# Phaken/graph-embeddings

Hardware: AMD Instinct MI355X
Metric: GloVe pair-updates/sec at dim=200 (higher is better)
Workload: dtype f32

## Files before the change

graph-embeddings_amd/csrc/ge_layout.h:

```cpp
#pragma once
#include "ge_common.h"
#include <vector>

namespace ge {

constexpr int LAYOUT_CHUNK = 128;

struct LayoutRequest {
    int32_t V, row_begin, row_end;
    int64_t N;
    int32_t cost;
    double  xmax;
    int32_t hot_columns;
    double  hot_theta;
    double  stale_budget;
    int32_t flush_every;
    int32_t workers;
    int32_t shared_rows;
    int32_t pack_rows;
    bool    want_hub_index;
    bool    device_input;
    int32_t tile_g;
    int32_t tile_force;
    int32_t tile_workers;
    int32_t panels;
    int32_t panel_blocks;
    int32_t blocks;
};

struct BlockedLayout {
    int32_t *bA = nullptr, *bB = nullptr, *border = nullptr;
    double  *L = nullptr;
    float   *W = nullptr;
    int32_t *cstart = nullptr;
    int32_t *cmeta = nullptr;
    int32_t *tcols = nullptr;
    int32_t *tlim = nullptr;
    int64_t P = 0, n_chunks = 0, n_hchunks = 0;
    int64_t n_tchunks = 0, tile_nnz = 0, tile_visits = 0;
    int32_t tile_g = 0, tile_cols = 0, n_tgroups = 0;
    int32_t *prow0 = nullptr, *prows = nullptr, *ppos = nullptr;
    int64_t n_pchunks = 0, panel_nnz = 0, panel_visits = 0;
// ... 20 lines not shown
```

graph-embeddings_amd/csrc/glove.hip:

```cpp

#include "ge_common.h"
#include "ge_coo.h"
#include "ge_glove_internal.h"
#include "ge_javarand.h"
#include "ge_cost.h"
#include "ge_exact.h"
#include "ge_strata.h"
#include "ge_wave.h"
#include "ge_layout.h"

#include <algorithm>
#include <cmath>
#include <cstdlib>
#include <cstring>
#include <chrono>
#include <memory>
#include <new>
#include <type_traits>
#include <vector>

namespace {

enum { ORDER_IDENTITY = 0, ORDER_PERM = 1, ORDER_BIJECTION = 2 };

// ... 191 lines not shown
    __builtin_amdgcn_s_waitcnt(0xC07F);
    __builtin_amdgcn_s_barrier();
    asm volatile("" ::: "memory");
}

constexpr int RUN_CHUNK = 128;
constexpr int KEY_PAD = 0x7FFFFFFF;
constexpr int TILE_N_AFTER = 4;

enum { PAIR_MEM = 0, PAIR_LDS = 1 };
struct PanelLink {
    const int32_t *rows;
    int32_t n_rows;
    int32_t lag;
    float *nextA, *nextB;
};
template <int G, int SRC, int SINK>
__device__ __forceinline__ void tile_chunk(const GloveParams &p, const int32_t c_lo, const int32_t c_len, const int32_t grp,
                                           float *const setA, float *const setB, float *const tr_c, float *const tr_g,
                                           int32_t *const stg, double &cost_acc, const PanelLink &pl, const int lane) {
    constexpr bool PIPE = SRC == PAIR_LDS || SINK == PAIR_LDS;
    constexpr int N_AFTER = SINK == PAIR_MEM ? TILE_N_AFTER : TILE_N_AFTER - 2;
    static_assert(G >= 2 && G <= 8, "two to eight resident columns");
    const int32_t D = p.D, DS = p.DS;
    const uint32_t row_bytes = (uint32_t)p.RW * 4u;
    const int bl_lane = (D / 4) & 63;
    const bool inr = lane * 4 < D, is_bl = lane == bl_lane;
    const float lr = p.lr;
    constexpr int IMG_G = 256;
    auto rl = [&](float v) { return __builtin_bit_cast(float, __builtin_amdgcn_readlane(__builtin_bit_cast(int, v), bl_lane)); };

    int s_lane = lane;
    asm volatile("" : "+v"(s_lane));
#pragma unroll
    for (int q = 0; q < 2; ++q) {
        const int e = q * 64 + s_lane;
        if (e < c_len) {
// ... 6 lines not shown
    __builtin_amdgcn_fence(__ATOMIC_RELEASE, "wavefront");
    __builtin_amdgcn_wave_barrier();
    __builtin_amdgcn_fence(__ATOMIC_ACQUIRE, "wavefront");
    auto staged = [&](int what, int e) { return rfl(stg[what * RUN_CHUNK + rfl(e)]); };
    auto row_at = [&](int e) { return staged(0, e); };

    auto request = [&](float *img, int32_t row, bool live) {
        const uint32_t rbytes = live ? row_bytes : 0u;
        load_to_lds<16>(make_rsrc(p.focus + (int64_t)row * DS, rbytes), img, lane * 16);
        load_to_lds<16>(make_rsrc(p.gsf + (int64_t)row * DS, rbytes), img + IMG_G, lane * 16);
        asm volatile("" ::: "memory");
    };
    int32_t n_row = 0;
    if constexpr (!PIPE) n_row = row_at(0);
    else if constexpr (SRC == PAIR_MEM) n_row = rfl(pl.rows[0]);
    if constexpr (SRC == PAIR_MEM) request(setA, n_row, true);

    float4 a[G], ga[G], a0[G], ga0[G];
    int32_t col[G], lim[G], cnt[G];
    auto ctx_rsrc = [&](int32_t c) { return make_rsrc(p.context + (int64_t)(c < 0 ? 0 : c) * DS, c < 0 ? 0u : row_bytes); };
    auto gsc_rsrc = [&](int32_t c) { return make_rsrc(p.gsc + (int64_t)(c < 0 ? 0 : c) * DS, c < 0 ? 0u : row_bytes); };
#pragma unroll
    for (int s = 0; s < G; ++s) {
        col[s] = rfl(p.tcols[(int64_t)grp * G + s]); lim[s] = rfl(p.tlim[(int64_t)grp * G + s]); cnt[s] = 0;
    }
#pragma unroll
    for (int s = 0; s < G; ++s) {
        a[s] = buf_load<4, AUX_SC1>(ctx_rsrc(col[s]), lane * 16);
        ga[s] = buf_load<4, AUX_SC1>(gsc_rsrc(col[s]), lane * 16);
    }
#pragma unroll
// ... 90 lines not shown
        bool more;
        if constexpr (!PIPE) {
            row = n_row;
            nxt = pos + 1;
            for (;;) {
                more = nxt < c_len;
                n_row = more ? row_at(nxt) : 0;
                if (!more || n_row != row) break;
                ++nxt;
            }
        } else {
            row = rfl(pl.rows[ri]);
            nxt = pos;
            while (nxt < c_len && row_at(nxt) == row) ++nxt;
            more = ri + 1 < pl.n_rows;
            if constexpr (SRC == PAIR_MEM) n_row = more ? rfl(pl.rows[ri + 1]) : 0;
        }
        const float *const img = decltype(CUR)::value ? setB : setA;
        if constexpr (SRC == PAIR_MEM) {
            request(decltype(CUR)::value ? setA : setB, n_row, more);
            __builtin_amdgcn_s_waitcnt(wait_vmcnt(N_AFTER));
        }
        asm volatile("" ::: "memory");
        b = *reinterpret_cast<const float4 *>(img + lane * 4);
        gb = *reinterpret_cast<const float4 *>(img + IMG_G + lane * 4);
        bb = rl(b.x); gbb = rl(gb.x);
        for (int e = pos; e < nxt; ++e) {
            const int s = staged(1, e);
            const float w = __builtin_bit_cast(float, staged(2, e));
            const unsigned lo = (unsigned)rfl(stg[3 * RUN_CHUNK + 2 * rfl(e)]), hi = (unsigned)rfl(stg[3 * RUN_CHUNK + 2 * rfl(e) + 1]);
            const double l = __builtin_bit_cast(double, ((unsigned long long)hi << 32) | lo);
            update(s, w, l);
        }
        float4 ob = b, ogb = gb;
        if (!inr) {
            ob = float4{0.0f, 0.0f, 0.0f, 0.0f}; ogb = ob;
            if (is_bl) { ob.x = bb; ogb.x = gbb; }
        }
        if constexpr (SINK == PAIR_MEM) {
            buf_store<4>(ob, make_rsrc(p.focus + (int64_t)row * DS, row_bytes), lane * 16);
// ... 18 lines not shown
        for (int ri = 0; ri < pl.n_rows; ri += 2) {
            walk_row(IMG_A, ri);
            lds_barrier();
            if (ri + 1 < pl.n_rows) {
                walk_row(IMG_B, ri + 1);
                lds_barrier();
            }
        }
        for (int i = pl.lag; i < 3; ++i) lds_barrier();
    }
#pragma nounroll
    for (int s = 0; s < G; ++s)
        for_slot(s, [&](auto S) { constexpr int q = decltype(S)::value; if (cnt[q] > 0) publish(col[q], a[q], ga[q], a0[q], ga0[q]); });
}

template <int VW, int NCH, int OPT, bool EMB16, bool FAT, int TG, bool PANELS = false>
__device__ __forceinline__ void epoch_walk(const GloveParams &p, const int32_t n_workers) {
    using VT = typename Vec<VW>::T;
    static_assert(!EMB16 || VW == 4, "bf16 embeddings need dim % 4 == 0");
    constexpr bool MOM = OPT != GE_OPT_ADAGRAD;
    int tid = (int)threadIdx.x;
    uint32_t sr_state = 0x9E3779B9u * (uint32_t)(threadIdx.x + 1) + (uint32_t)blockIdx.x * 0x85EBCA6Bu + p.bij_key[0];
    auto emb_rsrc = [&](float *base, int64_t id) {
        if constexpr (EMB16) return make_rsrc(reinterpret_cast<uint16_t *>(base) + id * p.ES, (uint32_t)p.D * 2u);
        else return make_rsrc(base + id * p.DS, (uint32_t)p.RW * 4u);
    };
    auto emb_load = [&](__amdgpu_buffer_rsrc_t rs, int q) -> VT {
        if constexpr (EMB16) return widen_bf16x4(buf_load<2, AUX_SC1>(rs, ((tid & 63) + q * 64) * 8));
        else return buf_load<VW, AUX_SC1>(rs, ((tid & 63) + q * 64) * VW * 4);
    };
    auto emb_store = [&](VT v, __amdgpu_buffer_rsrc_t rs, int q) {
// ... 59 lines not shown
            }
            __syncthreads();
            const int32_t tk = rfl(s_pticket);
            if (tk < 0) break;
            uint32_t x = (uint32_t)tk;
            do { x = bij_mix(x, p.pbij_mask, p.pbij_shift, p.bij_key); } while (x >= (uint32_t)n_pchunks);
            const int32_t pc = rfl((int)x);
            const int32_t r0 = rfl(p.prow0[pc]), nr = rfl(p.prow0[pc + 1]) - r0;
            if (tid < nr) s_prow[tid] = p.prows[r0 + tid];
            if (tid + 256 < nr && tid + 256 < 4 * RUN_CHUNK) s_prow[tid + 256] = p.prows[r0 + tid + 256];
            if (tid == 0) s_pn = nr < 4 * RUN_CHUNK ? nr : 4 * RUN_CHUNK;
            __syncthreads();
            const int32_t *const pp = p.ppos + (int64_t)pc * 9;
            const int32_t grp = rfl(pp[0]) * 4 + wib, c_lo = rfl(pp[1 + 2 * wib]), c_len = rfl(pp[2 + 2 * wib]);
            const int nx = wib < 3 ? wib + 1 : 0;
            const PanelLink pl{s_prow, rfl(s_pn), wib, s_setA + nx * SET_FLOATS, s_setB + nx * SET_FLOATS};
            float *const tr_c = s_tr[wib][0], *const tr_g = s_tr[wib][1];
            float *const setA = s_setA + wib * SET_FLOATS, *const setB = s_setB + wib * SET_FLOATS;
            if (wib == 0) tile_chunk<TG, PAIR_MEM, PAIR_LDS>(p, c_lo, c_len, grp, setA, setB, tr_c, tr_g, s_stage[wib], cost_acc, pl, tid & 63);
            else if (wib < 3) tile_chunk<TG, PAIR_LDS, PAIR_LDS>(p, c_lo, c_len, grp, setA, setB, tr_c, tr_g, s_stage[wib], cost_acc, pl, tid & 63);
            else tile_chunk<TG, PAIR_LDS, PAIR_MEM>(p, c_lo, c_len, grp, setA, setB, tr_c, tr_g, s_stage[wib], cost_acc, pl, tid & 63);
        }
        s_pcost[wib] = cost_acc;
        __syncthreads();
        if (wib == 0) cost_acc = ((s_pcost[0] + s_pcost[1]) + s_pcost[2]) + s_pcost[3];
        else cost_acc = 0.0;
        continue;
    }
    if (wave >= n_workers) continue;
    }
    const int lane = tid & 63;
    float *const setA = s_setA + (tid >> 6) * SET_FLOATS, *const setB = s_setB + (tid >> 6) * SET_FLOATS;
    bool inr[NCH];
#pragma unroll
// ... 379 lines not shown
    }
    if ((tid & 63) == 0 && cost_acc != 0.0) atomicAdd(p.cost_out, cost_acc);
}

template <int VW, int NCH, int OPT, bool EMB16, bool FAT>
__global__ __launch_bounds__(256, (NCH == 1 && VW == 4 && OPT == GE_OPT_ADAGRAD) ? 5 : 1) void k_adagrad_runs(GloveParams p, int32_t n_workers) {
    epoch_walk<VW, NCH, OPT, EMB16, FAT, 0>(p, n_workers);
}
constexpr int TILE_G = 4;
template <int G>
__global__ __launch_bounds__(256, 3) void k_epoch_tiles(GloveParams p, int32_t n_workers) {
    epoch_walk<4, 1, GE_OPT_ADAGRAD, false, true, G>(p, n_workers);
}
__global__ __launch_bounds__(256, 3) void k_epoch_panels(GloveParams p, int32_t n_workers) {
    epoch_walk<4, 1, GE_OPT_ADAGRAD, false, true, TILE_G, true>(p, n_workers);
}

__global__ __launch_bounds__(256) void k_probe_records(float *tab, int64_t rows, int64_t ds, int32_t rec_bytes, int32_t iters, uint32_t seed) {
    const int lane = threadIdx.x & 63;
    uint32_t x = (uint32_t)(blockIdx.x * 4 + (threadIdx.x >> 6)) * 0x9E3779B1u + seed;
    for (int it = 0; it < iters; ++it) {
        x = x * 1664525u + 1013904223u;
        const int64_t r = (int64_t)(((uint64_t)(x >> 4) * (uint64_t)rows) >> 28);
        const __amdgpu_buffer_rsrc_t rs = make_rsrc(tab + r * ds, (uint32_t)rec_bytes);
        float4 v[4];
#pragma unroll
        for (int q = 0; q < 4; ++q) v[q] = buf_load<4, AUX_SC1>(rs, (lane + q * 64) * 16);
#pragma unroll
        for (int q = 0; q < 4; ++q) buf_store<4>(v[q], rs, (lane + q * 64) * 16);
    }
// ... 298 lines not shown
    if (cfg->cost != GE_COST_GLOVE && cfg->cost != GE_COST_PGLOVE) return ge::fail(GE_ERR_ARG, "Invalid cost function %d", cfg->cost);
    if (cfg->opt < GE_OPT_ADAGRAD || cfg->opt > GE_OPT_AMSGRAD) return ge::fail(GE_ERR_ARG, "Invalid optimization method %d", cfg->opt);
    if (cfg->threads < 1) return ge::fail(GE_ERR_ARG, "threads must be >= 1");
    if (cfg->mode != GE_MODE_HOGWILD && cfg->mode != GE_MODE_DETERMINISTIC && cfg->mode != GE_MODE_STRATIFIED) return ge::fail(GE_ERR_ARG, "invalid mode %d", cfg->mode);
    if (cfg->strata < 0 || cfg->strata > 2048) return ge::fail(GE_ERR_ARG, "strata must lie in [0, 2048] (got %d; 0 = the default for the matrix)", cfg->strata);
    if (cfg->strata != 0 && cfg->mode != GE_MODE_STRATIFIED) return ge::fail(GE_ERR_ARG, "strata = %d needs mode = GE_MODE_STRATIFIED", cfg->strata);
    if (cfg->shuffle < GE_SHUFFLE_JAVA || cfg->shuffle > GE_SHUFFLE_NONE) return ge::fail(GE_ERR_ARG, "invalid shuffle %d", cfg->shuffle);
    if (cfg->mode == GE_MODE_STRATIFIED && cfg->shuffle == GE_SHUFFLE_JAVA)
        return ge::fail(GE_ERR_ARG, "the stratified mode cannot follow a global Fisher-Yates order: shuffle must be device or none");
    if (cfg->workers < -(1 << 20)) return ge::fail(GE_ERR_ARG, "workers out of range");
    if (cfg->emb_dtype != GE_DTYPE_F32 && cfg->emb_dtype != GE_DTYPE_BF16) return ge::fail(GE_ERR_ARG, "invalid emb_dtype %d", cfg->emb_dtype);
    const bool emb16 = cfg->emb_dtype == GE_DTYPE_BF16;
    if (emb16 && (cfg->mode != GE_MODE_HOGWILD || cfg->shuffle != GE_SHUFFLE_DEVICE || cfg->opt != GE_OPT_ADAGRAD || cfg->dim % 4 != 0))
        return ge::fail(GE_ERR_ARG, "bf16 embeddings need mode=hogwild, shuffle=device, opt=adagrad and dim %% 4 == 0 (the reference path is fp32)");
    if (cfg->hot_columns < GE_HOT_AUTO || cfg->hot_columns > GE_HOT_ALL) return ge::fail(GE_ERR_ARG, "invalid hot_columns %d", cfg->hot_columns);
    if (cfg->hot_theta < 0 || cfg->stale_budget < 0 || cfg->flush_every < 0 || cfg->blocks_per_cu < 0 || (cfg->layout_flags & ~511) != 0)
        return ge::fail(GE_ERR_ARG, "invalid tuning fields (hot_theta %g, stale_budget %g, flush_every %d, blocks_per_cu %d, layout_flags %d)",
                        (double)cfg->hot_theta, (double)cfg->stale_budget, cfg->flush_every, cfg->blocks_per_cu, cfg->layout_flags);
    int32_t rb = cfg->row_begin, re = cfg->row_end;
    if (rb == 0 && re == 0) re = cfg->vocab_size;
    if (rb < 0 || re > cfg->vocab_size || rb >= re) return ge::fail(GE_ERR_ARG, "invalid row range [%d,%d)", rb, re);
    const bool will_block = cfg->mode == GE_MODE_HOGWILD && cfg->shuffle == GE_SHUFFLE_DEVICE;
    if (!will_block)
        for (int64_t k = 0; k < cfg->nnz; ++k) {
            if (I[k] < rb || I[k] >= re) return ge::fail(GE_ERR_ARG, "I[%lld]=%d outside owned rows [%d,%d)", (long long)k, I[k], rb, re);
            if (J[k] < 0 || J[k] >= cfg->vocab_size) return ge::fail(GE_ERR_ARG, "J[%lld]=%d outside [0,%d)", (long long)k, J[k], cfg->vocab_size);
        }
    *rb_out = rb; *re_out = re;
    return GE_OK;
}

// ... 104 lines not shown
    blocks = std::min<int64_t>(blocks, std::max<int64_t>(1, N / 2048 / groups_per_block));
    w.blocks = (int)std::max<int64_t>(blocks, 1);
    w.workers = w.blocks * 4;
    if (cfg.workers > 0) {
        w.workers = (int)std::min<int64_t>(cfg.workers, (int64_t)h->num_cus * 32);
        w.blocks = (w.workers + 3) / 4;
    } else if (cfg.workers < 0) {
        w.blocks = (int)std::max<int64_t>(1, (int64_t)w.blocks - (-(int64_t)cfg.workers + 3) / 4);
        w.workers = w.blocks * 4;
    }
    return w;
}
void take_plan(ge_glove *h, const WorkerPlan &w) { h->hw_blocks_per_cu = w.blocks_per_cu; h->hw_blocks = w.blocks; h->hw_workers = w.workers; }
void plan_workers(ge_glove *h) { take_plan(h, plan_workers_of(h, h->hw.fn)); }

bool tiles_forced(const ge_glove_cfg &cfg) {
    const bool panels_asked = (cfg.layout_flags & (GE_LAYOUT_HUB_PANELS | GE_LAYOUT_NO_HUB_PANELS)) == GE_LAYOUT_HUB_PANELS;
    return (cfg.layout_flags & GE_LAYOUT_HUB_TILES) != 0 || (panels_asked && cfg.nnz < ((int64_t)1 << 25));
}
bool tiles_possible(const ge_glove *h) {
    const ge_glove_cfg &cfg = h->cfg;
    if (cfg.layout_flags & GE_LAYOUT_NO_HUB_TILES) return false;
    if (h->emb16 || cfg.opt != GE_OPT_ADAGRAD || !h->hw.fat || h->hw.vw != 4 || h->hw.nch != 1) return false;
    if (cfg.shuffle != GE_SHUFFLE_DEVICE || h->rows != cfg.vocab_size) return false;
    return tiles_forced(cfg) || cfg.nnz >= ((int64_t)1 << 25);
}
bool panels_possible(const ge_glove *h) {
    const ge_glove_cfg &cfg = h->cfg;
    if ((cfg.layout_flags & GE_LAYOUT_NO_HUB_PANELS) || !tiles_possible(h)) return false;
    return (cfg.layout_flags & GE_LAYOUT_HUB_PANELS) != 0 || cfg.nnz >= ((int64_t)1 << 25);
}

ge_status plan_epoch_layout(ge_glove *h, const int32_t *I, const int32_t *J, const float *X, bool device_input) {
    const ge_glove_cfg &cfg = h->cfg;
    const int32_t V = cfg.vocab_size;
    const int64_t N = cfg.nnz;
    const double theta = cfg.hot_theta > 0 ? (double)cfg.hot_theta : 0.25;
    const double stale_budget = cfg.stale_budget > 0 ? (double)cfg.stale_budget : 2000.0;
    h->blocked = cfg.shuffle == GE_SHUFFLE_DEVICE;
    if (h->blocked) {
        ge::LayoutRequest rq{};
        rq.V = V; rq.row_begin = cfg.row_begin; rq.row_end = cfg.row_end; rq.N = N; rq.cost = cfg.cost; rq.xmax = cfg.xmax;
        rq.hot_columns = cfg.hot_columns; rq.hot_theta = theta; rq.stale_budget = stale_budget; rq.flush_every = cfg.flush_every;
        rq.workers = h->hw_workers;
        rq.shared_rows = (cfg.layout_flags & GE_LAYOUT_PLAIN_LONG_ROWS) ? 0 : 1;
        rq.pack_rows = (cfg.layout_flags & GE_LAYOUT_FIXED_CUTS) ? 0 : 1;
        rq.want_hub_index = h->emb16;
        rq.device_input = device_input;
        const hogwild_fn tile_fn = k_epoch_tiles<TILE_G>;
        WorkerPlan tile_plan{};
        if (tiles_possible(h)) {
            tile_plan = plan_workers_of(h, tile_fn);
            rq.tile_g = TILE_G; rq.tile_force = tiles_forced(cfg) ? 1 : 0; rq.tile_workers = tile_plan.workers;
            if (panels_possible(h)) {
                rq.panels = 1; rq.blocks = tile_plan.blocks;
                if (const char *e = std::getenv("GE_PANEL_BLOCKS")) rq.panel_blocks = std::max(0, std::atoi(e));
            }
        }
        GE_CHECK(ge::build_blocked_layout(rq, I, J, X, h->stream, &h->lay));
        if (h->lay.n_tchunks > 0 || h->lay.n_pchunks > 0) { h->hw.fn = h->lay.n_pchunks > 0 ? (hogwild_fn)k_epoch_panels : tile_fn; take_plan(h, tile_plan); }
        h->n_chunks = h->lay.n_chunks; h->n_hchunks = h->lay.n_hchunks; h->n_tchunks = h->lay.n_tchunks; h->n_pchunks = h->lay.n_pchunks;
        h->hot_cols = h->lay.hot_cols; h->hot_nnz = h->lay.hot_nnz; h->hot_threshold = h->lay.hot_threshold;
        h->flush_every = h->lay.flush_min;
        if (h->emb16) { h->host_hub_index.swap(h->lay.hub_index); h->n_hub = h->lay.n_hub; }
        return GE_OK;
    }
    std::vector<int32_t> cnt((size_t)V, 0);
    std::vector<uint8_t> hotcol((size_t)V, 0);
    if (N > 0 && cfg.hot_columns != GE_HOT_NONE) {
        const int64_t thr = cfg.hot_columns == GE_HOT_ALL ? 0
                          : std::max<int64_t>(2, (int64_t)std::ceil(theta * (double)N / (double)h->hw_workers));
        for (int64_t k = 0; k < N; ++k) ++cnt[(size_t)J[k]];
        for (int32_t v = 0; v < V; ++v)
            if (cnt[(size_t)v] >= thr && cnt[(size_t)v] > 0) { hotcol[(size_t)v] = 1; ++h->hot_cols; h->hot_nnz += cnt[(size_t)v]; }
        h->hot_threshold = thr;
// ... 484 lines not shown
```

graph-embeddings_amd/csrc/glove_layout.hip:

```cpp
#include "ge_layout.h"
#include "ge_cost.h"

#include <algorithm>
#include <cmath>
#include <chrono>
#include <cstdio>
#include <cstdlib>
#include <cstring>
#include <vector>

#include <rocprim/device/device_radix_sort.hpp>

namespace {

__device__ __forceinline__ int lane_id() { return threadIdx.x & 63; }

__device__ __forceinline__ void wave_count(int32_t *cnt, int32_t key, bool active) {
    bool todo = active;
    for (;;) {
        const unsigned long long m = __ballot(todo);
        if (!m) break;
        const int leader = __ffsll((long long)m) - 1;
        const int32_t k0 = __shfl(key, leader, 64);
        const bool same = todo && key == k0;
// ... 170 lines not shown
    std::vector<int32_t> hubsR;
    int32_t n_tgroups = 0;
    out->n_tchunks = 0; out->tile_nnz = 0; out->tile_visits = 0; out->tile_g = 0; out->tile_cols = 0; out->n_tgroups = 0;
    out->n_pchunks = 0; out->panel_nnz = 0; out->panel_visits = 0; out->n_panels = 0; out->panel_cols = 0; out->panel_blocks = 0;
    out->host_prow0.clear(); out->host_ppos.clear();
    int32_t n_panels = 0;
    auto hub_threshold = [&](int32_t wk) -> int64_t {
        int64_t thr = rq.hot_columns == GE_HOT_ALL ? 0
                    : std::max<int64_t>(2, (int64_t)std::ceil(rq.hot_theta * (double)N / (double)std::max(wk, 1)));
        if (rq.row_end - rq.row_begin < V) thr = std::min(thr, heavy_thr);
        return thr;
    };
    if (N > 0 && rq.hot_columns != GE_HOT_NONE) {
        if (G >= 2) {
            const int64_t thr_t = hub_threshold(rq.workers);
            std::vector<int32_t> el;
            for (int32_t v = 0; v < V; ++v)
                if (cnt[(size_t)v] >= thr_t && cnt[(size_t)v] > 0 && (rq.tile_force || (int64_t)cnt[(size_t)v] * 8 >= (int64_t)rows)) el.push_back(v);
            std::stable_sort(el.begin(), el.end(), [&](int32_t a, int32_t b) { return cnt[(size_t)a] > cnt[(size_t)b]; });
            size_t n_el = el.size();
            if (n_el % (size_t)G == 1) --n_el;
            const uint64_t groups = (n_el + (size_t)G - 1) / (size_t)G;
            if (groups * (uint64_t)rows * (uint64_t)G + (uint64_t)V + (uint64_t)rows >= ((uint64_t)1 << 32) || groups * (uint64_t)rows > ((uint64_t)1 << 28)) {
                if (rq.tile_force && n_el >= 2)
                    return ge::fail(GE_ERR_ARG, "layout hub_tiles: %llu column groups x %d rows are too many for the tile build (forced tiles are for small matrices)",
                                    (unsigned long long)groups, rows);
                n_el = 0;
            }
            if (n_el >= 2) {
                n_tgroups = (int32_t)groups;
                tile_slot.assign((size_t)V, -1); tcols.assign((size_t)n_tgroups * G, -1); tlim.assign((size_t)n_tgroups * G, LAYOUT_CHUNK);
                if (rq.panels && G == 4) n_panels = (int32_t)(n_el / (size_t)G / 4);
                for (size_t k = 0; k < n_el; ++k) {
                    tile_slot[(size_t)el[k]] = (int32_t)k; tcols[k] = el[k];
                    (k < (size_t)n_panels * 16 ? out->panel_nnz : out->tile_nnz) += cnt[(size_t)el[k]];
                }
                out->n_panels = n_panels; out->panel_cols = n_panels * 16;
                out->tile_g = G; out->tile_cols = (int32_t)n_el - out->panel_cols; out->n_tgroups = n_tgroups;
// ... 104 lines not shown
            close();
            for (int w = 0; w < 4; ++w)
                for (size_t c = first; c < ppos.size() / 9; ++c) { sub_start.push_back(ppos[c * 9 + 1 + 2 * w]); sub_meta.push_back(pn * 4 + w); }
            if (gpos[3] != gbase) return ge::fail(GE_ERR_STATE, "internal: panel %d covers %lld of its positions", pn, (long long)(gpos[3] - gbase));
        }
        sub_start.push_back((int32_t)nP);
        if (gbase != nP) return ge::fail(GE_ERR_STATE, "internal: panel counts cover %lld of %lld nonzeros", (long long)gbase, (long long)nP);
    }
    out->n_pchunks = (int64_t)ppos.size() / 9;
    if (n_panels > 0) {
        int32_t pb = rq.panel_blocks;
        const double w_panels = PANEL_STEP_COST * (double)(panel_steps + 3 * out->n_pchunks), w_main = (double)(N - nP) / 4.0;
        if (clk.on) std::fprintf(stderr, "[ge_glove_create]   layout: panel steps %lld, chunks %lld, main nonzeros %lld\n", (long long)panel_steps, (long long)out->n_pchunks, (long long)(N - nP));
        if (pb <= 0) pb = (int32_t)std::lround(w_panels / std::max(w_panels + w_main, 1.0) * (double)rq.blocks);
        out->panel_blocks = std::max(1, std::min(pb, std::max(rq.blocks, 1)));
        for (int32_t pn = 0; pn < n_panels; ++pn) {
            const double K = std::max(1.0, (double)out->panel_blocks * (double)panel_chunks[(size_t)pn] / (double)std::max<int64_t>(out->n_pchunks, 1));
            const int32_t m = rq.flush_every > 0 ? std::min<int32_t>(rq.flush_every, LAYOUT_CHUNK)
                                                 : (int32_t)std::min<double>(LAYOUT_CHUNK, std::max<double>(4.0, std::floor(rq.stale_budget / K)));
            for (int k = 0; k < 16; ++k) tlim[(size_t)pn * 16 + k] = m;
            out->flush_min = std::min(out->flush_min, m);
        }
    }
    {
        int64_t placed = nP;
        for (int32_t g = 4 * n_panels; g < n_tgroups; ++g) {
            int32_t used = 0;
            for (int s = 0; s < G; ++s) if (tcols[(size_t)g * G + s] >= 0) ++used;
            int32_t fill = 0;
            auto close = [&]() {
// ... 171 lines not shown
```

graph-embeddings_amd/geglove/capi.py:

```python
import ctypes as C
import os

_HERE = os.path.dirname(os.path.abspath(__file__))
LIB_PATH = os.path.join(os.path.dirname(_HERE), "lib", "libgeglove.so")

GE_OK, GE_ERR_ARG, GE_ERR_OOM, GE_ERR_HIP, GE_ERR_STATE, GE_ERR_OVERFLOW = 0, -1, -2, -3, -4, -5
GE_COST_GLOVE, GE_COST_PGLOVE = 0, 1
GE_OPT_ADAGRAD, GE_OPT_ADAM, GE_OPT_AMSGRAD = 0, 1, 2
GE_NORM_NONE, GE_NORM_UNITY, GE_NORM_COUNTS = 0, 1, 2
GE_MODE_HOGWILD, GE_MODE_DETERMINISTIC, GE_MODE_STRATIFIED = 0, 1, 2
GE_ARITH_JAVA, GE_ARITH_FP32 = 0, 1
GE_SHUFFLE_JAVA, GE_SHUFFLE_DEVICE, GE_SHUFFLE_NONE = 0, 1, 2
GE_HOT_AUTO, GE_HOT_NONE, GE_HOT_ALL = 0, 1, 2
GE_DTYPE_F32, GE_DTYPE_BF16 = 0, 1
GE_LAYOUT_FIXED_CUTS, GE_LAYOUT_PLAIN_LONG_ROWS, GE_LAYOUT_SEPARATE_TABLES, GE_LAYOUT_PACKED_RECORDS, GE_LAYOUT_FIRST_PLACEMENT = 1, 2, 4, 8, 16
GE_LAYOUT_HUB_TILES, GE_LAYOUT_NO_HUB_TILES = 32, 64
GE_LAYOUT_HUB_PANELS, GE_LAYOUT_NO_HUB_PANELS = 128, 256
(GE_STATE_FOCUS, GE_STATE_CONTEXT, GE_STATE_FBIAS, GE_STATE_CBIAS, GE_STATE_GSQ_FOCUS,
 GE_STATE_GSQ_CONTEXT, GE_STATE_GSQ_FBIAS, GE_STATE_GSQ_CBIAS, GE_STATE_M2_FOCUS, GE_STATE_M2_CONTEXT,
 GE_STATE_M2_FBIAS, GE_STATE_M2_CBIAS) = range(12)
STATE_NAMES = ("focus", "context", "fbias", "cbias", "gsq_focus", "gsq_context", "gsq_fbias", "gsq_cbias")
M2_NAMES = ("m2_focus", "m2_context", "m2_fbias", "m2_cbias")
ALL_STATE_NAMES = STATE_NAMES + M2_NAMES

SYMBOLS = (
    "ge_glove_cfg_default", "ge_glove_create", "ge_glove_epoch", "ge_glove_extract_f32",
    "ge_glove_extract_f64", "ge_glove_get_state", "ge_glove_set_state", "ge_glove_device_ptr",
    "ge_glove_epoch_order", "ge_glove_get_perm", "ge_glove_rng_state", "ge_glove_last_kernel_ms", "ge_glove_get_info", "ge_glove_tile_info", "ge_glove_panel_info", "ge_glove_destroy",
    "ge_bca_build", "ge_coo_get", "ge_coo_destroy", "ge_exchange_turn_bf16", "ge_glove_context_layout",
    "ge_local_group_create", "ge_local_group_destroy", "ge_local_group_abort", "ge_rccl_unique_id", "ge_rccl_selftest", "ge_sync_cfg_size", "ge_sync_create", "ge_sync_begin", "ge_sync_finish", "ge_sync_turn", "ge_sync_sync",
    "ge_sync_epoch", "ge_sync_hub_rows", "ge_sync_hub_exchange", "ge_sync_hub_exchange_live", "ge_sync_live_rows", "ge_sync_hub_plan", "ge_sync_replicate", "ge_sync_allreduce_f64", "ge_sync_destroy",
    "ge_sim_cfg_default", "ge_sim_cfg_size", "ge_sim_pattern_supported", "ge_similarity_pairs", "ge_sim_pairs_get", "ge_sim_pairs_destroy", "ge_copy_bandwidth", "ge_last_error", "ge_version", "ge_glove_cfg_size", "ge_glove_info_size", "ge_bca_cfg_size", "ge_device_count",
# ... 908 lines not shown
```

graph-embeddings_amd/geglove/host.py:

```python
import ctypes as C
import math
import os

import numpy as np

from . import capi


def _p(a, ct):
    return a.ctypes.data_as(C.POINTER(ct))


class InvalidConfigurationException(Exception):

    def __init__(self, message):
        super().__init__("Invalid configuration: " + message)


class GloveCost:
    kind = capi.GE_COST_GLOVE


class PGloveCost:
    kind = capi.GE_COST_PGLOVE
# ... 183 lines not shown
def device_arith(dev):
    word = str(dev.get("arith", "java")).lower()
    if word not in _ARITH:
        raise InvalidConfigurationException("Invalid device.arith, choose one of: java, fp32")
    if word == "fp32" and str(dev.get("mode", "hogwild")).lower() != "stratified":
        raise InvalidConfigurationException("device.arith: fp32 needs device.mode: stratified")
    return _ARITH[word]


_MODES = {"hogwild": capi.GE_MODE_HOGWILD, "deterministic": capi.GE_MODE_DETERMINISTIC, "stratified": capi.GE_MODE_STRATIFIED}
_HOT = {"auto": capi.GE_HOT_AUTO, "none": capi.GE_HOT_NONE, "all": capi.GE_HOT_ALL}
_SHUFFLES = {"java": capi.GE_SHUFFLE_JAVA, "device": capi.GE_SHUFFLE_DEVICE, "none": capi.GE_SHUFFLE_NONE}
_LAYOUT = {"default": 0, "fixed_cuts": capi.GE_LAYOUT_FIXED_CUTS, "plain_long_rows": capi.GE_LAYOUT_PLAIN_LONG_ROWS,
           "separate_tables": capi.GE_LAYOUT_SEPARATE_TABLES, "packed_records": capi.GE_LAYOUT_PACKED_RECORDS,
           "first_placement": capi.GE_LAYOUT_FIRST_PLACEMENT, "hub_tiles": capi.GE_LAYOUT_HUB_TILES, "no_hub_tiles": capi.GE_LAYOUT_NO_HUB_TILES,
           "hub_panels": capi.GE_LAYOUT_HUB_PANELS, "no_hub_panels": capi.GE_LAYOUT_NO_HUB_PANELS}


class Adagrad:
    OPT = capi.GE_OPT_ADAGRAD
    NAME = "Adagrad"
    """`new Adagrad(coMatrix, config, costFunction)` + IOptimizer (J/opt/grad/Adagrad.java,
    J/opt/Optimizer.java, J/opt/IOptimizer.java:6-11) over ge_glove_*.

    Extra keyword arguments override config.device.* : mode, shuffle, seed, device, stream,
    row_range (multi-GPU sharding), learning_rate.  coMatrix may be a DeviceCooMatrix (a ge_coo handle).
    """

    def __init__(self, coMatrix, config, costFunction, **kw):
        dev = dict(config.device)
        dev.update({k: v for k, v in kw.items() if v is not None})
# ... 277 lines not shown
```

graph-embeddings_amd/host/ge_host.hpp:

```cpp
#pragma once

#include <algorithm>
#include <cerrno>
#include <charconv>
#include <cmath>
#include <cstdint>
#include <cstdio>
#include <cstdlib>
#include <cstring>
#include <ctime>
#include <filesystem>
#include <fstream>
#include <map>
#include <set>
#include <iterator>
#include <limits>
#include <condition_variable>
#include <memory>
#include <mutex>
#include <sstream>
#include <stdexcept>
#include <string>
#include <thread>
#include <unordered_map>
// ... 346 lines not shown
                    else if (q.first == "bca_table_slots") c.device.bca_table_slots = (long long)num(&q.second);
                    else if (q.first == "bca_pool_entries") c.device.bca_pool_entries = (long long)num(&q.second);
                    else if (q.first == "layout") {
                        std::vector<std::string> names; bool present = false;
                        if (q.second.kind == YNode::List) strlist(&q.second, present, names); else names.push_back(q.second.scalar);
                        for (auto &nm : names) {
                            if (nm == "fixed_cuts") c.device.layout_flags |= GE_LAYOUT_FIXED_CUTS;
                            else if (nm == "plain_long_rows") c.device.layout_flags |= GE_LAYOUT_PLAIN_LONG_ROWS;
                            else if (nm == "separate_tables") c.device.layout_flags |= GE_LAYOUT_SEPARATE_TABLES;
                            else if (nm == "packed_records") c.device.layout_flags |= GE_LAYOUT_PACKED_RECORDS;
                            else if (nm == "first_placement") c.device.layout_flags |= GE_LAYOUT_FIRST_PLACEMENT;
                            else if (nm == "hub_tiles") c.device.layout_flags |= GE_LAYOUT_HUB_TILES;
                            else if (nm == "no_hub_tiles") c.device.layout_flags |= GE_LAYOUT_NO_HUB_TILES;
                            else if (nm == "hub_panels") c.device.layout_flags |= GE_LAYOUT_HUB_PANELS;
                            else if (nm == "no_hub_panels") c.device.layout_flags |= GE_LAYOUT_NO_HUB_PANELS;
                            else if (!nm.empty() && nm != "default") throw std::invalid_argument("device.layout: unknown flag " + nm);
                        }
                    }
                }
            } else c.ignored_keys.push_back(k);
        }
        return c;
    }

    static void check(const Configuration &c) {
        const bool hasBca = c.bca.present && c.bca.alpha > 0 && c.bca.epsilon > 0;
        const bool hasOut = c.output.present && (c.output.has_predicate || c.output.has_blank || c.output.has_uri || c.output.has_literal);
        if (!(c.dim > 0)) throw InvalidConfigurationException("No dimension specified");
        if (c.graph.empty()) throw InvalidConfigurationException("No input graph specified");
        if (c.method.empty()) throw InvalidConfigurationException("Invalid method, choose one of: glove, pglove");
// ... 1250 lines not shown
```

include/geglove.h:

```cpp
#ifndef GEGLOVE_H
#define GEGLOVE_H

#include <stdint.h>

#ifdef __cplusplus
extern "C" {
#endif

typedef int32_t ge_status;
enum {
    GE_OK           =  0,
    GE_ERR_ARG      = -1,
    GE_ERR_OOM      = -2,
    GE_ERR_HIP      = -3,
    GE_ERR_STATE    = -4,
    GE_ERR_OVERFLOW = -5
};

enum { GE_COST_GLOVE = 0, GE_COST_PGLOVE = 1 };
enum { GE_OPT_ADAGRAD = 0, GE_OPT_ADAM = 1, GE_OPT_AMSGRAD = 2 };
enum { GE_NORM_NONE = 0, GE_NORM_UNITY = 1, GE_NORM_COUNTS = 2 };

enum { GE_MODE_HOGWILD = 0, GE_MODE_DETERMINISTIC = 1, GE_MODE_STRATIFIED = 2 };

// ... 39 lines not shown
    void   *stream;
    int32_t row_begin;
    int32_t row_end;
    int32_t hot_columns;
    int32_t workers;
    int32_t emb_dtype;
    float   hot_theta;
    float   stale_budget;
    int32_t flush_every;
    int32_t blocks_per_cu;
    int32_t layout_flags;
    int32_t strata;
} ge_glove_cfg;

enum { GE_LAYOUT_FIXED_CUTS = 1, GE_LAYOUT_PLAIN_LONG_ROWS = 2, GE_LAYOUT_SEPARATE_TABLES = 4, GE_LAYOUT_PACKED_RECORDS = 8, GE_LAYOUT_FIRST_PLACEMENT = 16,
       GE_LAYOUT_HUB_TILES = 32, GE_LAYOUT_NO_HUB_TILES = 64, GE_LAYOUT_HUB_PANELS = 128, GE_LAYOUT_NO_HUB_PANELS = 256 };

typedef struct {
    int32_t group_width;
    int32_t vector_width;
    int32_t chunks_per_lane;
    int32_t blocks;
    int32_t groups_in_flight;
    int32_t hot_columns;
    int64_t hot_nonzeros;
    int64_t hot_threshold;
    int64_t chunks;
    int64_t hub_chunks;
    int64_t long_rows;
    int64_t shared_chunks;
    int32_t flush_min;
// ... 308 lines not shown
```

Before: 2.210 billion.

## Add deep prefetch ring for panel stage-0 rows and widen panel hub admission

Adds a k_epoch_ring kernel whose first panel stage keeps a ring of KD+1 focus-row images in shared memory and issues row loads KD rows ahead, instead of double-buffering one row ahead. This is meant to hide global-memory latency on focus/gradient row fetches. The layout builder also admits sparser hub columns into panels (a density divisor of 16 instead of 8, rounded to multiples of 16 under size limits), shifting more nonzeros into the panel path. It is the default whenever panels are possible and hub_panels is not forced. The cost is extra LDS per workgroup, which may reduce occupancy.

```diff
diff --git a/graph-embeddings_amd/csrc/ge_layout.h b/graph-embeddings_amd/csrc/ge_layout.h
--- a/graph-embeddings_amd/csrc/ge_layout.h
+++ b/graph-embeddings_amd/csrc/ge_layout.h
@@ -26,6 +26,7 @@
     int32_t panels;
     int32_t panel_blocks;
     int32_t blocks;
+    int32_t panel_div;
 };
 
 struct BlockedLayout {
diff --git a/graph-embeddings_amd/csrc/glove.hip b/graph-embeddings_amd/csrc/glove.hip
--- a/graph-embeddings_amd/csrc/glove.hip
+++ b/graph-embeddings_amd/csrc/glove.hip
@@ -229,13 +229,17 @@
     int32_t n_rows;
     int32_t lag;
     float *nextA, *nextB;
+    float *ring;
 };
-template <int G, int SRC, int SINK>
+constexpr int RING_IMG = 512;
+template <int G, int SRC, int SINK, int KD = 1>
 __device__ __forceinline__ void tile_chunk(const GloveParams &p, const int32_t c_lo, const int32_t c_len, const int32_t grp,
                                            float *const setA, float *const setB, float *const tr_c, float *const tr_g,
                                            int32_t *const stg, double &cost_acc, const PanelLink &pl, const int lane) {
     constexpr bool PIPE = SRC == PAIR_LDS || SINK == PAIR_LDS;
-    constexpr int N_AFTER = SINK == PAIR_MEM ? TILE_N_AFTER : TILE_N_AFTER - 2;
+    constexpr int N_AFTER = KD > 1 ? 2 * KD : SINK == PAIR_MEM ? TILE_N_AFTER : TILE_N_AFTER - 2;
+    static_assert(KD == 1 || (KD >= 2 && SRC == PAIR_MEM && SINK == PAIR_LDS), "the request ring is stage 0's: it stores nothing to memory");
+    static_assert(N_AFTER < 64, "vmcnt is a 6-bit counter");
     static_assert(G >= 2 && G <= 8, "two to eight resident columns");
     const int32_t D = p.D, DS = p.DS;
     const uint32_t row_bytes = (uint32_t)p.RW * 4u;
@@ -272,7 +276,16 @@
     int32_t n_row = 0;
     if constexpr (!PIPE) n_row = row_at(0);
     else if constexpr (SRC == PAIR_MEM) n_row = rfl(pl.rows[0]);
-    if constexpr (SRC == PAIR_MEM) request(setA, n_row, true);
+    int ring_cur = 0;
+    if constexpr (KD == 1) {
+        if constexpr (SRC == PAIR_MEM) request(setA, n_row, true);
+    } else {
+#pragma unroll
+        for (int q = 0; q < KD; ++q) {
+            const bool live = q < pl.n_rows;
+            request(pl.ring + q * RING_IMG, live ? rfl(pl.rows[q]) : 0, live);
+        }
+    }
 
     float4 a[G], ga[G], a0[G], ga0[G];
     int32_t col[G], lim[G], cnt[G];
@@ -393,16 +406,30 @@
             nxt = pos;
             while (nxt < c_len && row_at(nxt) == row) ++nxt;
             more = ri + 1 < pl.n_rows;
-            if constexpr (SRC == PAIR_MEM) n_row = more ? rfl(pl.rows[ri + 1]) : 0;
+            if constexpr (SRC == PAIR_MEM && KD == 1) n_row = more ? rfl(pl.rows[ri + 1]) : 0;
         }
         const float *const img = decltype(CUR)::value ? setB : setA;
+        if constexpr (KD > 1) {
+            const bool ahead = ri + KD < pl.n_rows;
+            const int32_t a_row = ahead ? rfl(pl.rows[ri + KD]) : 0;
+            request(pl.ring + (ring_cur == 0 ? KD : ring_cur - 1) * RING_IMG, a_row, ahead);
+            __builtin_amdgcn_s_waitcnt(wait_vmcnt(N_AFTER));
+            const uint32_t at = (uint32_t)(uintptr_t)GE_LDS(pl.ring + ring_cur * RING_IMG) + (uint32_t)lane * 16u;
+            ge_i4 rb, rgb;
+            asm volatile("ds_read_b128 %0, %2\n\tds_read_b128 %1, %2 offset:1024\n\ts_waitcnt lgkmcnt(0)"
+                         : "=&v"(rb), "=&v"(rgb) : "v"(at) : "memory");
+            __builtin_memcpy(&b, &rb, 16); __builtin_memcpy(&gb, &rgb, 16);
+            ring_cur = ring_cur == KD ? 0 : ring_cur + 1;
+        } else
         if constexpr (SRC == PAIR_MEM) {
             request(decltype(CUR)::value ? setA : setB, n_row, more);
             __builtin_amdgcn_s_waitcnt(wait_vmcnt(N_AFTER));
         }
         asm volatile("" ::: "memory");
-        b = *reinterpret_cast<const float4 *>(img + lane * 4);
-        gb = *reinterpret_cast<const float4 *>(img + IMG_G + lane * 4);
+        if constexpr (KD == 1) {
+            b = *reinterpret_cast<const float4 *>(img + lane * 4);
+            gb = *reinterpret_cast<const float4 *>(img + IMG_G + lane * 4);
+        }
         bb = rl(b.x); gbb = rl(gb.x);
         for (int e = pos; e < nxt; ++e) {
             const int s = staged(1, e);
@@ -451,7 +478,7 @@
         for_slot(s, [&](auto S) { constexpr int q = decltype(S)::value; if (cnt[q] > 0) publish(col[q], a[q], ga[q], a0[q], ga0[q]); });
 }
 
-template <int VW, int NCH, int OPT, bool EMB16, bool FAT, int TG, bool PANELS = false>
+template <int VW, int NCH, int OPT, bool EMB16, bool FAT, int TG, bool PANELS = false, int KD = 1>
 __device__ __forceinline__ void epoch_walk(const GloveParams &p, const int32_t n_workers) {
     using VT = typename Vec<VW>::T;
     static_assert(!EMB16 || VW == 4, "bf16 embeddings need dim % 4 == 0");
@@ -541,10 +568,16 @@
             const int32_t *const pp = p.ppos + (int64_t)pc * 9;
             const int32_t grp = rfl(pp[0]) * 4 + wib, c_lo = rfl(pp[1 + 2 * wib]), c_len = rfl(pp[2 + 2 * wib]);
             const int nx = wib < 3 ? wib + 1 : 0;
-            const PanelLink pl{s_prow, rfl(s_pn), wib, s_setA + nx * SET_FLOATS, s_setB + nx * SET_FLOATS};
+            float *ring = nullptr;
+            if constexpr (KD > 1) {
+                static_assert(SET_FLOATS == RING_IMG && IMG_G * 2 == RING_IMG, "an image of the ring is a focus pair's");
+                __shared__ float s_ring[(KD + 1) * RING_IMG];
+                ring = s_ring;
+            }
+            const PanelLink pl{s_prow, rfl(s_pn), wib, s_setA + nx * SET_FLOATS, s_setB + nx * SET_FLOATS, ring};
             float *const tr_c = s_tr[wib][0], *const tr_g = s_tr[wib][1];
             float *const setA = s_setA + wib * SET_FLOATS, *const setB = s_setB + wib * SET_FLOATS;
-            if (wib == 0) tile_chunk<TG, PAIR_MEM, PAIR_LDS>(p, c_lo, c_len, grp, setA, setB, tr_c, tr_g, s_stage[wib], cost_acc, pl, tid & 63);
+            if (wib == 0) tile_chunk<TG, PAIR_MEM, PAIR_LDS, KD>(p, c_lo, c_len, grp, setA, setB, tr_c, tr_g, s_stage[wib], cost_acc, pl, tid & 63);
             else if (wib < 3) tile_chunk<TG, PAIR_LDS, PAIR_LDS>(p, c_lo, c_len, grp, setA, setB, tr_c, tr_g, s_stage[wib], cost_acc, pl, tid & 63);
             else tile_chunk<TG, PAIR_LDS, PAIR_MEM>(p, c_lo, c_len, grp, setA, setB, tr_c, tr_g, s_stage[wib], cost_acc, pl, tid & 63);
         }
@@ -954,6 +987,14 @@
 }
 __global__ __launch_bounds__(256, 3) void k_epoch_panels(GloveParams p, int32_t n_workers) {
     epoch_walk<4, 1, GE_OPT_ADAGRAD, false, true, TILE_G, true>(p, n_workers);
+}
+#ifndef GE_RING_K
+#define GE_RING_K 2
+#endif
+constexpr int RING_K = GE_RING_K;
+static_assert(RING_K >= 2 && 2 * RING_K < 64, "vmcnt is a 6-bit counter");
+__global__ __launch_bounds__(256, 3) void k_epoch_ring(GloveParams p, int32_t n_workers) {
+    epoch_walk<4, 1, GE_OPT_ADAGRAD, false, true, TILE_G, true, RING_K>(p, n_workers);
 }
 
 __global__ __launch_bounds__(256) void k_probe_records(float *tab, int64_t rows, int64_t ds, int32_t rec_bytes, int32_t iters, uint32_t seed) {
@@ -1282,7 +1323,7 @@
     if (emb16 && (cfg->mode != GE_MODE_HOGWILD || cfg->shuffle != GE_SHUFFLE_DEVICE || cfg->opt != GE_OPT_ADAGRAD || cfg->dim % 4 != 0))
         return ge::fail(GE_ERR_ARG, "bf16 embeddings need mode=hogwild, shuffle=device, opt=adagrad and dim %% 4 == 0 (the reference path is fp32)");
     if (cfg->hot_columns < GE_HOT_AUTO || cfg->hot_columns > GE_HOT_ALL) return ge::fail(GE_ERR_ARG, "invalid hot_columns %d", cfg->hot_columns);
-    if (cfg->hot_theta < 0 || cfg->stale_budget < 0 || cfg->flush_every < 0 || cfg->blocks_per_cu < 0 || (cfg->layout_flags & ~511) != 0)
+    if (cfg->hot_theta < 0 || cfg->stale_budget < 0 || cfg->flush_every < 0 || cfg->blocks_per_cu < 0 || (cfg->layout_flags & ~2047) != 0)
         return ge::fail(GE_ERR_ARG, "invalid tuning fields (hot_theta %g, stale_budget %g, flush_every %d, blocks_per_cu %d, layout_flags %d)",
                         (double)cfg->hot_theta, (double)cfg->stale_budget, cfg->flush_every, cfg->blocks_per_cu, cfg->layout_flags);
     int32_t rb = cfg->row_begin, re = cfg->row_end;
@@ -1417,8 +1458,9 @@
 void take_plan(ge_glove *h, const WorkerPlan &w) { h->hw_blocks_per_cu = w.blocks_per_cu; h->hw_blocks = w.blocks; h->hw_workers = w.workers; }
 void plan_workers(ge_glove *h) { take_plan(h, plan_workers_of(h, h->hw.fn)); }
 
+bool deep_asked(const ge_glove_cfg &cfg) { return (cfg.layout_flags & GE_LAYOUT_DEEP_PANELS) != 0; }
 bool tiles_forced(const ge_glove_cfg &cfg) {
-    const bool panels_asked = (cfg.layout_flags & (GE_LAYOUT_HUB_PANELS | GE_LAYOUT_NO_HUB_PANELS)) == GE_LAYOUT_HUB_PANELS;
+    const bool panels_asked = ((cfg.layout_flags & GE_LAYOUT_HUB_PANELS) != 0 || deep_asked(cfg)) && (cfg.layout_flags & GE_LAYOUT_NO_HUB_PANELS) == 0;
     return (cfg.layout_flags & GE_LAYOUT_HUB_TILES) != 0 || (panels_asked && cfg.nnz < ((int64_t)1 << 25));
 }
 bool tiles_possible(const ge_glove *h) {
@@ -1431,8 +1473,14 @@
 bool panels_possible(const ge_glove *h) {
     const ge_glove_cfg &cfg = h->cfg;
     if ((cfg.layout_flags & GE_LAYOUT_NO_HUB_PANELS) || !tiles_possible(h)) return false;
-    return (cfg.layout_flags & GE_LAYOUT_HUB_PANELS) != 0 || cfg.nnz >= ((int64_t)1 << 25);
-}
+    return (cfg.layout_flags & GE_LAYOUT_HUB_PANELS) != 0 || deep_asked(cfg) || cfg.nnz >= ((int64_t)1 << 25);
+}
+bool ring_possible(const ge_glove *h) {
+    const ge_glove_cfg &cfg = h->cfg;
+    if ((cfg.layout_flags & GE_LAYOUT_NO_DEEP_PANELS) || !panels_possible(h)) return false;
+    return deep_asked(cfg) || (cfg.layout_flags & GE_LAYOUT_HUB_PANELS) == 0;
+}
+constexpr int PANEL_DENSITY_DIV = 16;
 
 ge_status plan_epoch_layout(ge_glove *h, const int32_t *I, const int32_t *J, const float *X, bool device_input) {
     const ge_glove_cfg &cfg = h->cfg;
@@ -1452,16 +1500,24 @@
         rq.device_input = device_input;
         const hogwild_fn tile_fn = k_epoch_tiles<TILE_G>;
         WorkerPlan tile_plan{};
+        bool ring = false;
         if (tiles_possible(h)) {
             tile_plan = plan_workers_of(h, tile_fn);
             rq.tile_g = TILE_G; rq.tile_force = tiles_forced(cfg) ? 1 : 0; rq.tile_workers = tile_plan.workers;
             if (panels_possible(h)) {
                 rq.panels = 1; rq.blocks = tile_plan.blocks;
                 if (const char *e = std::getenv("GE_PANEL_BLOCKS")) rq.panel_blocks = std::max(0, std::atoi(e));
+                if (ring_possible(h)) {
+                    ring = true;
+                    if (!rq.tile_force) {
+                        rq.panel_div = PANEL_DENSITY_DIV;
+                        if (const char *e = std::getenv("GE_PANEL_DENSITY_DIV")) rq.panel_div = std::max(8, std::atoi(e));
+                    }
+                }
             }
         }
         GE_CHECK(ge::build_blocked_layout(rq, I, J, X, h->stream, &h->lay));
-        if (h->lay.n_tchunks > 0 || h->lay.n_pchunks > 0) { h->hw.fn = h->lay.n_pchunks > 0 ? (hogwild_fn)k_epoch_panels : tile_fn; take_plan(h, tile_plan); }
+        if (h->lay.n_tchunks > 0 || h->lay.n_pchunks > 0) { h->hw.fn = h->lay.n_pchunks > 0 ? (ring ? (hogwild_fn)k_epoch_ring : (hogwild_fn)k_epoch_panels) : tile_fn; take_plan(h, tile_plan); }
         h->n_chunks = h->lay.n_chunks; h->n_hchunks = h->lay.n_hchunks; h->n_tchunks = h->lay.n_tchunks; h->n_pchunks = h->lay.n_pchunks;
         h->hot_cols = h->lay.hot_cols; h->hot_nnz = h->lay.hot_nnz; h->hot_threshold = h->lay.hot_threshold;
         h->flush_every = h->lay.flush_min;
diff --git a/graph-embeddings_amd/csrc/glove_layout.hip b/graph-embeddings_amd/csrc/glove_layout.hip
--- a/graph-embeddings_amd/csrc/glove_layout.hip
+++ b/graph-embeddings_amd/csrc/glove_layout.hip
@@ -208,14 +208,25 @@
     if (N > 0 && rq.hot_columns != GE_HOT_NONE) {
         if (G >= 2) {
             const int64_t thr_t = hub_threshold(rq.workers);
+            const int64_t div = (!rq.tile_force && rq.panels && G == 4 && rq.panel_div > 8) ? (int64_t)rq.panel_div : 8;
             std::vector<int32_t> el;
             for (int32_t v = 0; v < V; ++v)
-                if (cnt[(size_t)v] >= thr_t && cnt[(size_t)v] > 0 && (rq.tile_force || (int64_t)cnt[(size_t)v] * 8 >= (int64_t)rows)) el.push_back(v);
+                if (cnt[(size_t)v] >= thr_t && cnt[(size_t)v] > 0 && (rq.tile_force || (int64_t)cnt[(size_t)v] * div >= (int64_t)rows)) el.push_back(v);
             std::stable_sort(el.begin(), el.end(), [&](int32_t a, int32_t b) { return cnt[(size_t)a] > cnt[(size_t)b]; });
-            size_t n_el = el.size();
-            if (n_el % (size_t)G == 1) --n_el;
+            size_t n_dense = el.size();
+            if (div > 8) { n_dense = 0; while (n_dense < el.size() && (int64_t)cnt[(size_t)el[n_dense]] * 8 >= (int64_t)rows) ++n_dense; }
+            auto too_large = [&](uint64_t groups) {
+                return groups * (uint64_t)rows * (uint64_t)G + (uint64_t)V + (uint64_t)rows >= ((uint64_t)1 << 32) || groups * (uint64_t)rows > ((uint64_t)1 << 28);
+            };
+            size_t adm = el.size(), n_el = 0;
+            for (;;) {
+                n_el = std::max(adm / 16 * 16, n_dense);
+                if (n_el % (size_t)G == 1) --n_el;
+                if (adm <= n_dense || !too_large((n_el + (size_t)G - 1) / (size_t)G)) break;
+                adm = std::max(n_dense, adm / 16 * 16 - (adm % 16 == 0 ? 16 : 0));
+            }
             const uint64_t groups = (n_el + (size_t)G - 1) / (size_t)G;
-            if (groups * (uint64_t)rows * (uint64_t)G + (uint64_t)V + (uint64_t)rows >= ((uint64_t)1 << 32) || groups * (uint64_t)rows > ((uint64_t)1 << 28)) {
+            if (too_large(groups)) {
                 if (rq.tile_force && n_el >= 2)
                     return ge::fail(GE_ERR_ARG, "layout hub_tiles: %llu column groups x %d rows are too many for the tile build (forced tiles are for small matrices)",
                                     (unsigned long long)groups, rows);
@@ -350,6 +361,7 @@
         if (clk.on) std::fprintf(stderr, "[ge_glove_create]   layout: panel steps %lld, chunks %lld, main nonzeros %lld\n", (long long)panel_steps, (long long)out->n_pchunks, (long long)(N - nP));
         if (pb <= 0) pb = (int32_t)std::lround(w_panels / std::max(w_panels + w_main, 1.0) * (double)rq.blocks);
         out->panel_blocks = std::max(1, std::min(pb, std::max(rq.blocks, 1)));
+        if (clk.on) std::fprintf(stderr, "[ge_glove_create]   layout: %d panels, %d of %d workgroups start in the panel loop\n", n_panels, out->panel_blocks, rq.blocks);
         for (int32_t pn = 0; pn < n_panels; ++pn) {
             const double K = std::max(1.0, (double)out->panel_blocks * (double)panel_chunks[(size_t)pn] / (double)std::max<int64_t>(out->n_pchunks, 1));
             const int32_t m = rq.flush_every > 0 ? std::min<int32_t>(rq.flush_every, LAYOUT_CHUNK)
diff --git a/graph-embeddings_amd/geglove/capi.py b/graph-embeddings_amd/geglove/capi.py
--- a/graph-embeddings_amd/geglove/capi.py
+++ b/graph-embeddings_amd/geglove/capi.py
@@ -16,6 +16,7 @@
 GE_LAYOUT_FIXED_CUTS, GE_LAYOUT_PLAIN_LONG_ROWS, GE_LAYOUT_SEPARATE_TABLES, GE_LAYOUT_PACKED_RECORDS, GE_LAYOUT_FIRST_PLACEMENT = 1, 2, 4, 8, 16
 GE_LAYOUT_HUB_TILES, GE_LAYOUT_NO_HUB_TILES = 32, 64
 GE_LAYOUT_HUB_PANELS, GE_LAYOUT_NO_HUB_PANELS = 128, 256
+GE_LAYOUT_DEEP_PANELS, GE_LAYOUT_NO_DEEP_PANELS = 512, 1024
 (GE_STATE_FOCUS, GE_STATE_CONTEXT, GE_STATE_FBIAS, GE_STATE_CBIAS, GE_STATE_GSQ_FOCUS,
  GE_STATE_GSQ_CONTEXT, GE_STATE_GSQ_FBIAS, GE_STATE_GSQ_CBIAS, GE_STATE_M2_FOCUS, GE_STATE_M2_CONTEXT,
  GE_STATE_M2_FBIAS, GE_STATE_M2_CBIAS) = range(12)
diff --git a/graph-embeddings_amd/geglove/host.py b/graph-embeddings_amd/geglove/host.py
--- a/graph-embeddings_amd/geglove/host.py
+++ b/graph-embeddings_amd/geglove/host.py
@@ -221,7 +221,8 @@
 _LAYOUT = {"default": 0, "fixed_cuts": capi.GE_LAYOUT_FIXED_CUTS, "plain_long_rows": capi.GE_LAYOUT_PLAIN_LONG_ROWS,
            "separate_tables": capi.GE_LAYOUT_SEPARATE_TABLES, "packed_records": capi.GE_LAYOUT_PACKED_RECORDS,
            "first_placement": capi.GE_LAYOUT_FIRST_PLACEMENT, "hub_tiles": capi.GE_LAYOUT_HUB_TILES, "no_hub_tiles": capi.GE_LAYOUT_NO_HUB_TILES,
-           "hub_panels": capi.GE_LAYOUT_HUB_PANELS, "no_hub_panels": capi.GE_LAYOUT_NO_HUB_PANELS}
+           "hub_panels": capi.GE_LAYOUT_HUB_PANELS, "no_hub_panels": capi.GE_LAYOUT_NO_HUB_PANELS,
+           "deep_panels": capi.GE_LAYOUT_DEEP_PANELS, "no_deep_panels": capi.GE_LAYOUT_NO_DEEP_PANELS}
 
 
 class Adagrad:
diff --git a/graph-embeddings_amd/host/ge_host.hpp b/graph-embeddings_amd/host/ge_host.hpp
--- a/graph-embeddings_amd/host/ge_host.hpp
+++ b/graph-embeddings_amd/host/ge_host.hpp
@@ -384,6 +384,8 @@
                             else if (nm == "no_hub_tiles") c.device.layout_flags |= GE_LAYOUT_NO_HUB_TILES;
                             else if (nm == "hub_panels") c.device.layout_flags |= GE_LAYOUT_HUB_PANELS;
                             else if (nm == "no_hub_panels") c.device.layout_flags |= GE_LAYOUT_NO_HUB_PANELS;
+                            else if (nm == "deep_panels") c.device.layout_flags |= GE_LAYOUT_DEEP_PANELS;
+                            else if (nm == "no_deep_panels") c.device.layout_flags |= GE_LAYOUT_NO_DEEP_PANELS;
                             else if (!nm.empty() && nm != "default") throw std::invalid_argument("device.layout: unknown flag " + nm);
                         }
                     }
diff --git a/include/geglove.h b/include/geglove.h
--- a/include/geglove.h
+++ b/include/geglove.h
@@ -77,7 +77,8 @@
 } ge_glove_cfg;
 
 enum { GE_LAYOUT_FIXED_CUTS = 1, GE_LAYOUT_PLAIN_LONG_ROWS = 2, GE_LAYOUT_SEPARATE_TABLES = 4, GE_LAYOUT_PACKED_RECORDS = 8, GE_LAYOUT_FIRST_PLACEMENT = 16,
-       GE_LAYOUT_HUB_TILES = 32, GE_LAYOUT_NO_HUB_TILES = 64, GE_LAYOUT_HUB_PANELS = 128, GE_LAYOUT_NO_HUB_PANELS = 256 };
+       GE_LAYOUT_HUB_TILES = 32, GE_LAYOUT_NO_HUB_TILES = 64, GE_LAYOUT_HUB_PANELS = 128, GE_LAYOUT_NO_HUB_PANELS = 256,
+       GE_LAYOUT_DEEP_PANELS = 512, GE_LAYOUT_NO_DEEP_PANELS = 1024 };
 
 typedef struct {
     int32_t group_width;
```

Result: faster. 2.258 billion, median of 6 (+2.2%).
